# ChrisHekmanOtoy/opencl_render

Hardware: AMD Instinct MI355X
Metric: Mrays/s (primary rays; each also traces its shadow/bounce rays) at ms/frame = ms_per_step (higher is better)
Workload: dtype f32

## Files before the change

### opencl_render_amd/csrc/rt_wavefront.hip

```cpp
#include "rt_devfuncs.h"
#include "rt_launch.h"
#include "rt_ray_clip.h"

namespace {

enum { WS_RAY = 0, WS_SHADOW = 1 };

__device__ __forceinline__ float4 pack4(V3 v, float w) { return make_float4(v.x, v.y, v.z, w); }
__device__ __forceinline__ V3 xyz(float4 v) { return mk(v.x, v.y, v.z); }

__device__ __forceinline__ void store_single_sample(const RtDevScene &S, uint32_t localPixel, V3 c)
{
    const uint32_t slot = localPixel / RT_TILE_PIXELS, inTile = localPixel % RT_TILE_PIXELS;
    uint16_t *planes = S.tileBuf + (size_t)slot * 3 * RT_TILE_PIXELS + inTile;
    uint32_t samples = S.sampleDivisor;
    asm volatile("" : "+s"(samples));
    const float scale = (float)(0xFFFF) / (float)samples;
    planes[0] = (uint16_t)sat_add_u16(0, c.x, scale);
    planes[RT_TILE_PIXELS] = (uint16_t)sat_add_u16(0, c.y, scale);
    planes[2 * RT_TILE_PIXELS] = (uint16_t)sat_add_u16(0, c.z, scale);
}

__device__ __forceinline__ uint32_t wave_append(uint32_t *counter, bool want)
{
    const unsigned long long mask = __ballot(want);
    if (mask == 0) return 0;
    const uint32_t lane = __lane_id();
    const int leader = __ffsll((long long)mask) - 1;
    uint32_t base = 0;
    if ((int)lane == leader) base = atomicAdd(counter, (uint32_t)__popcll(mask));
    base = __shfl(base, leader, 64);
    return base + (uint32_t)__popcll(mask & ((1ull << lane) - 1ull));
}

__device__ __forceinline__ void wave_append2(uint32_t *counterA, bool wantA, uint32_t *counterB, bool wantB, uint32_t &posA, uint32_t &posB)
{
    const unsigned long long maskA = __ballot(wantA), maskB = __ballot(wantB);
    const uint32_t lane = __lane_id();
    uint32_t base = 0;
    const uint32_t n = (lane == 0u) ? (uint32_t)__popcll(maskA) : (uint32_t)__popcll(maskB);
    if (lane < 2u && n != 0u) base = atomicAdd(lane == 0u ? counterA : counterB, n);
    const unsigned long long below = (1ull << lane) - 1ull;
    posA = (uint32_t)__shfl((int)base, 0, 64) + (uint32_t)__popcll(maskA & below);
    posB = (uint32_t)__shfl((int)base, 1, 64) + (uint32_t)__popcll(maskB & below);
}

__device__ __forceinline__ bool tri_rec_test_flat(const float4 r0, const float4 r1, const float4 r2, const float4 r3, V3 o, V3 d, float tmin,
                                                  float tmax, float &t, float &l1, float &l2)
{
    const V3 a = mk(r0.x, r0.y, r0.z), ab = mk(r0.w, r1.x, r1.y), ac = mk(r1.z, r1.w, r2.x), n = mk(r2.y, r2.z, r2.w);
    const V3 ao = sub3(o, a);
    t = -dot3(n, ao) / dot3(n, d);
    const V3 ap = sub3(along(o, t, d), a);
    const float ap_ab = dot3(ap, ab);
    const float ap_ac = dot3(ap, ac);
    l1 = (r3.y * ap_ac - r3.z * ap_ab) * r3.w;
    l2 = (r3.y * ap_ab - r3.x * ap_ac) * r3.w;
    return (tmin < t) & (t < tmax) & (0 <= l1) & (0 <= l2) & (l1 + l2 <= 1.f);
}
// ... 78 lines not shown
}

#if defined(RT_DIAG_STAMPS) || defined(RT_DIAG_LOGIC)
__device__ __forceinline__ unsigned long long diag_stamp()
{
    unsigned long long t;
    asm volatile("s_memtime %0\n\ts_waitcnt lgkmcnt(0)" : "=s"(t)::"memory");
    return t;
}
#endif

}

template <bool PASSES>
__device__ __forceinline__ void wf_primary_body(const RtDevScene &S, const RtWavefront &W, uint32_t *passBuf)
{
    const uint32_t slot = blockIdx.x >> 6, patch = blockIdx.x & 63;
    const uint32_t lane = threadIdx.x & 63, wave = threadIdx.x >> 6;
    const uint32_t lx = (patch & 7) * RT_PATCH + (wave & 1) * 8 + (lane & 7);
    const uint32_t ly = (patch >> 3) * RT_PATCH + (wave >> 1) * 8 + (lane >> 3);
    const uint32_t tile = S.tileIds[slot];
    const uint32_t gx = (tile % S.tilesX) * RT_TILE + lx;
    const uint32_t gy = (tile / S.tilesX) * RT_TILE + ly;
    const uint32_t sb = blockIdx.y;
    const bool valid = gx < S.width && gy < S.height;

    uint32_t hit_tri = RT_NONE;
    float hit_t = 0.f, hit_l1 = 0.f, hit_l2 = 0.f;
    uint64_t rng = 0;
    V3 dir = mk(0.f, 0.f, 0.f);
    const uint32_t localPixel = slot * RT_TILE_PIXELS + ly * RT_TILE + lx;
    const uint32_t outSlot = localPixel * W.samplesInBatch + sb;
    if (valid) {
        const uint32_t pixel = gy * S.width + gx;
        rng = (uint64_t)pixel * (uint64_t)S.seedStride + (uint64_t)(S.sampleFirst + W.sampleBase + sb + 1);
        const V3 lr = ld3(S.lr), tb = ld3(S.tb);
        dir = ld3(S.topLeft);
        float k = (float)gx + rand01(rng);
        dir.x += lr.x * k; dir.y += lr.y * k; dir.z += lr.z * k;
        k = (float)gy + rand01(rng);
        dir.x += tb.x * k; dir.y += tb.y * k; dir.z += tb.z * k;
        hit_tri = camera_scan(S, localPixel, ld3(S.eye), dir, 0.f, RT_INF, RT_NONE, hit_t, hit_l1, hit_l2);
        if (hit_tri == RT_NONE) {
            if (S.directStore == 1u) store_single_sample(S, localPixel, mk(0.f, 0.f, 0.f));
            else W.sampleOut[outSlot] = make_float4(0.f, 0.f, 0.f, 0.f);
        }
    }
    const bool born = valid && hit_tri != RT_NONE;
    const uint32_t shard = (blockIdx.x + blockIdx.y * gridDim.x) % RT_WF_SHARDS;
    const uint32_t a = shard * W.shardCap + wave_append(&W.ctl[RT_WF_CTL_COUNTS + shard], born);
    if (born) {
        W.rng[a] = rng;
        W.meta[a] = make_uint4(outSlot, localPixel, 0u | (1u << 4) | ((uint32_t)WS_RAY << 8), hit_tri);
        W.ring[(size_t)a * (RT_RING * 3) + 1] = pack4(dir, __uint_as_float(RT_NONE));
        W.res[a] = make_uint4(hit_tri, __float_as_uint(hit_t), __float_as_uint(hit_l1), __float_as_uint(hit_l2));
    }
    if (PASSES && valid) {
        uint32_t *pass = passBuf + (size_t)slot * RT_PASS_WORDS * RT_TILE_PIXELS + ly * RT_TILE + lx;
        if (S.sampleCount == 1u) pass[RT_PASS_HITS * RT_TILE_PIXELS] = born ? 1u : 0u;
        else if (born) __hip_atomic_fetch_add(pass + RT_PASS_HITS * RT_TILE_PIXELS, 1u, __ATOMIC_RELAXED, __HIP_MEMORY_SCOPE_AGENT);
        if (W.sampleBase + sb == 0u) {
            const float depth = born ? hit_t * sqrt_rn(dot3(dir, dir)) : RT_INF;
            pass[RT_PASS_DEPTH * RT_TILE_PIXELS] = __float_as_uint(depth);
            pass[RT_PASS_TRIANGLE * RT_TILE_PIXELS] = hit_tri;
        }
    }
}

__global__ __launch_bounds__(256) void wf_primary_kernel(const RtDevScene S, const RtWavefront W) { wf_primary_body<false>(S, W, nullptr); }
__global__ __launch_bounds__(256) void wf_primary_passes_kernel(const RtDevScene S, const RtWavefront W, uint32_t *passBuf)
{
    wf_primary_body<true>(S, W, passBuf);
}

__global__ __launch_bounds__(256) void wf_surface_passes_kernel(const RtDevScene S, const RtWavefront W, float *surfBuf)
{
    __shared__ Shared sh;
    for (int i = threadIdx.x; i < 3 * (RT_GRID_DIV + 1); i += 256) (&sh.planes[0][0])[i] = S.boxMin[i];
    sh.unit255[threadIdx.x] = (float)threadIdx.x / 255.f;
    __syncthreads();
    const uint32_t slot = blockIdx.x >> 6, patch = blockIdx.x & 63;
    const uint32_t lane = threadIdx.x & 63, wave = threadIdx.x >> 6;
    const uint32_t lx = (patch & 7) * RT_PATCH + (wave & 1) * 8 + (lane & 7);
    const uint32_t ly = (patch >> 3) * RT_PATCH + (wave >> 1) * 8 + (lane >> 3);
    const uint32_t tile = S.tileIds[slot];
    const uint32_t gx = (tile % S.tilesX) * RT_TILE + lx;
    const uint32_t gy = (tile / S.tilesX) * RT_TILE + ly;
    if (gx >= S.width || gy >= S.height) return;

    const uint32_t localPixel = slot * RT_TILE_PIXELS + ly * RT_TILE + lx;
    float *sums = surfBuf + (size_t)slot * RT_SURF_WORDS * RT_TILE_PIXELS + ly * RT_TILE + lx;
    float acc[RT_SURF_WORDS];
#pragma unroll
    for (int k = 0; k < RT_SURF_WORDS; ++k) acc[k] = W.sampleBase == 0u ? 0.f : sums[k * RT_TILE_PIXELS];
    const uint32_t pixel = gy * S.width + gx;
    const V3 eye = ld3(S.eye), lr = ld3(S.lr), tb = ld3(S.tb), topLeft = ld3(S.topLeft);
    Counters cn;
    for (uint32_t sb = 0; sb < W.samplesInBatch; ++sb) {
        uint64_t rng = (uint64_t)pixel * (uint64_t)S.seedStride + (uint64_t)(S.sampleFirst + W.sampleBase + sb + 1);
        V3 dir = topLeft;
        float k = (float)gx + rand01(rng);
        dir.x += lr.x * k; dir.y += lr.y * k; dir.z += lr.z * k;
        k = (float)gy + rand01(rng);
        dir.x += tb.x * k; dir.y += tb.y * k; dir.z += tb.z * k;
        float hit_t = 0.f, hit_l1 = 0.f, hit_l2 = 0.f;
        const uint32_t hit_tri = camera_scan(S, localPixel, eye, dir, 0.f, RT_INF, RT_NONE, hit_t, hit_l1, hit_l2);
        V3 n = mk(0.f, 0.f, 0.f), albedo = mk(0.f, 0.f, 0.f);
// ... 187 lines not shown
    const float4 *sp = reinterpret_cast<const float4 *>(S.triShade + 24 * (size_t)tri);
    const float4 s0 = sp[0], s1 = sp[1], s2 = sp[2], s3 = sp[3], s4 = sp[4], s5 = sp[5];
    row.a = reinterpret_cast<const float4 *>(S.triRec)[4 * (size_t)tri];
    row.v[0] = s0.x; row.v[1] = s0.y; row.v[2] = s0.z; row.v[3] = s0.w; row.v[4] = s1.x; row.v[5] = s1.y; row.v[6] = s1.z; row.v[7] = s1.w;
    row.v[8] = s2.x; row.v[9] = s2.y; row.v[10] = s2.z; row.v[11] = s2.w; row.v[12] = s3.x; row.v[13] = s3.y; row.v[14] = s3.z; row.v[15] = s3.w;
    row.v[16] = s4.x; row.v[17] = s4.y; row.v[18] = s4.z; row.v[19] = s4.w; row.v[20] = s5.x; row.v[21] = s5.y; row.v[22] = s5.z; row.v[23] = s5.w;
    row.tri = tri;
}

template <bool FIRST, bool ORDERED, bool LEAN>
__global__ __launch_bounds__(256, LEAN ? (FIRST ? RT_WF_LOGIC_WAVES_LEAN_FIRST : RT_WF_LOGIC_WAVES_LEAN)
                                       : (FIRST ? (ORDERED ? RT_WF_LOGIC_WAVES_FIRST_ORDERED : RT_WF_LOGIC_WAVES_FIRST) : RT_WF_LOGIC_WAVES)) void wf_logic_kernel(const RtDevScene S, const RtWavefront W, const uint32_t round,
                                                                                                             const uint32_t slicesIn, const RtRoundMode next)
{
    constexpr bool SHADE = false;
    const RtShadeList L{ nullptr, nullptr };
#include "rt_wf_logic_body.h"
}

#ifndef RT_WF_ANSWER_WAVES
#define RT_WF_ANSWER_WAVES 8
#endif
__global__ __launch_bounds__(256, RT_WF_ANSWER_WAVES) void wf_answer_kernel(const RtDevScene S, const RtWavefront W, const uint32_t round, const uint32_t slicesIn,
                                                                            const RtShadeList L, const uint32_t shadeFollows)
{
    const uint32_t in = round & 1;
    const uint32_t *ctlIn = W.ctl + (round % 3) * RT_WF_CTL_WORDS;
    const uint32_t lane = threadIdx.x & 63, wave = threadIdx.x >> 6;
    const uint32_t waveId = (blockIdx.x * 256 + threadIdx.x) >> 6, waves = (gridDim.x * 256) >> 6;
    {
        const uint32_t gid = blockIdx.x * 256 + threadIdx.x;
        if (gid < RT_WF_CTL_WORDS) W.ctl[((round + 2) % 3) * RT_WF_CTL_WORDS + gid] = 0u;
        if (gid < RT_WF_SHARDS) L.count[((round + 2) % 3) * RT_WF_SHARDS + gid] = 0u;
    }
    if (blockIdx.x == gridDim.x - 1 && round < RT_WF_ROUND_LOG) log_round_rays(W, ctlIn, round, lane, wave);
    const uint32_t shard = __builtin_amdgcn_readfirstlane(waveId % slicesIn);
    const uint32_t total = __builtin_amdgcn_readfirstlane(ctlIn[RT_WF_CTL_COUNTS + shard]);
    const uint32_t sliceCapIn = W.capacity / slicesIn;
    uint32_t *listCount = L.count + (round % 3) * RT_WF_SHARDS + shard;
    const float4 lc = S.lightCount != 0u ? make_float4(S.lightCol[0], S.lightCol[1], S.lightCol[2], S.lightHalfAtt[0]) : make_float4(0.f, 0.f, 0.f, 0.f);
    for (uint32_t localChunk = __builtin_amdgcn_readfirstlane(waveId / slicesIn); localChunk * 64 < total; localChunk += waves / slicesIn) {
        const uint32_t local = localChunk * 64 + lane;
        const uint32_t q = shard * sliceCapIn + local;
        bool list = false, odd = false;
        uint32_t a = 0;
        unsigned long long listKey = ~0ull;
        if (local < total) {
            const uint2 who = W.pathOf[in][q];
            a = who.x;
            const unsigned long long key = W.hitKey[in][q];
            unsigned long long laKey = ~0ull;
            if (who.y != 0xffffffffu) laKey = W.hitKey[in][who.y];
            const uint4 meta = W.meta[a];
            V3 out = xyz(W.outc[a]);
            int head = (int)(meta.z & 15u);
            const int tail = (int)((meta.z >> 4) & 15u);
            const uint32_t stage = (meta.z >> 8) & 1u, laState = (meta.z >> 10) & 3u;
            const int laIndex = (int)((meta.z >> 12) & 15u);
            if (laState == 2u) laKey = W.laKey[a];
            bool finished = false;
            if (stage == WS_SHADOW) {
                const float4 sp = W.shP[a], sf = W.shFace[a];
                const float lmax = reinterpret_cast<const float *>(W.ent[in] + 4 * (size_t)q)[11];
                const V3 zero = mk(0.f, 0.f, 0.f);
                V3 face = xyz(sf), atten = mk(1.f, 1.f, 1.f);
                if (key != ~0ull) { atten.x *= zero.x; atten.y *= zero.y; atten.z *= zero.z; }
                class_light_accum(face, sp.w, sf.w != 0.f, lmax, lc, atten);
                class_shade_end(out, xyz(sp), face);
                head = (head + 1) % RT_RING;
                if (head == tail) finished = true;
                else if (laState != 0u && laIndex == head) {
                    if (laKey != ~0ull) { list = true; listKey = laKey; W.outc[a] = pack4(out, 0.f); }
                    else if ((head + 1) % RT_RING == tail) finished = true;
                    else odd = true;
                } else odd = true;
            } else if (laState != 0u) odd = true;
            else if (key != ~0ull) { list = true; listKey = key; }
            else if ((head + 1) % RT_RING == tail) finished = true;
            else odd = true;
            if (finished) {
                if (S.directStore == 1u) store_single_sample(S, meta.y, out);
                else W.sampleOut[meta.x] = pack4(out, 0.f);
            }
        }
        if (__ballot(odd) != 0ull && lane == 0u) atomicOr(W.hostStatus + RT_WF_STATUS_ERROR, RT_WF_ERR_SPLIT);
        if (!shadeFollows && __ballot(list) != 0ull && lane == 0u) atomicOr(W.hostStatus + RT_WF_STATUS_ERROR, RT_WF_ERR_GRID);
        const uint32_t at = wave_append(listCount, list);
        if (list) L.list[shard * sliceCapIn + at] = make_uint4(a, (uint32_t)listKey, (uint32_t)(listKey >> 32), 0u);
    }
}

template <bool ORDERED>
__global__ __launch_bounds__(256, RT_WF_LOGIC_WAVES_LEAN) void wf_shade_kernel(const RtDevScene S, const RtWavefront W, const uint32_t round, const uint32_t slicesIn,
                                                                              const RtRoundMode next, const RtShadeList L)
{
    constexpr bool FIRST = false, LEAN = true, SHADE = true;
#include "rt_wf_logic_body.h"
}

__device__ __forceinline__ uint32_t slice_first(const RtWavefront &W, uint32_t slices, uint32_t s)
{
    const uint32_t kind = (s >= slices) ? 1u : 0u, shard = s - kind * slices;
    return kind * W.capacity + shard * (W.capacity / slices);
}
__device__ __forceinline__ uint32_t slice_count(const uint32_t *ctl, uint32_t slices, uint32_t s)
{
    const uint32_t kind = (s >= slices) ? 1u : 0u, shard = s - kind * slices;
    return ctl[RT_WF_CTL_COUNTS + kind * RT_WF_SHARDS + shard];
}

__global__ __launch_bounds__(256) void wf_scatter_kernel(const RtWavefront W, const uint32_t round, const uint32_t slices)
{
    __shared__ uint32_t base[RT_WF_SORT_BINS * RT_WF_SORT_COPIES];
    __shared__ uint32_t longWave[4];
    uint32_t *ctl = W.ctl + (round % 3) * RT_WF_CTL_WORDS;
    const uint32_t lane = threadIdx.x & 63, wave = threadIdx.x >> 6;
// ... 1164 lines not shown
```

### opencl_render_amd/csrc/rt_wf_logic_body.h

```cpp
    __shared__ Shared sh;
    __shared__ float4 ltPosRadius[RT_WF_LIGHTS_LDS], ltDirSpread[RT_WF_LIGHTS_LDS], ltColHalf[RT_WF_LIGHTS_LDS];
    __shared__ int ltType[RT_WF_LIGHTS_LDS];
    __shared__ uint32_t waveHist[ORDERED ? 4 : 1][RT_WF_SORT_BINS], waveBase[ORDERED ? 4 : 1][RT_WF_SORT_BINS];
    __shared__ uint8_t cellLut[ORDERED ? 3 * 256 : 4];
    __shared__ uint8_t itemOwner[ORDERED ? 4 : 1][2 * 64 * (RT_WF_MAXSEG - 1)];
    __shared__ uint32_t itemWord[ORDERED ? 4 : 1][ORDERED ? 2 * 64 * (RT_WF_MAXSEG - 1) : 1];
    __shared__ float lutScale[3];
    static_assert(RT_WF_SORT_BINS == 64, "one class per lane");
    sh.unit255[threadIdx.x] = (float)threadIdx.x / 255.f;
    if (ORDERED) {
        float *pl = &sh.planes[0][0];
        for (int i = threadIdx.x; i < 3 * (RT_GRID_DIV + 1); i += 256) pl[i] = S.boxMin[i];
        waveHist[threadIdx.x >> 6][threadIdx.x & 63] = 0u;
        if (threadIdx.x < 3 * 256 / 4) reinterpret_cast<uint32_t *>(cellLut)[threadIdx.x] = reinterpret_cast<const uint32_t *>(S.cellLut)[threadIdx.x];
        if (threadIdx.x < 3) lutScale[threadIdx.x] = 256.f / (S.boxMin[threadIdx.x * (RT_GRID_DIV + 1) + RT_GRID_DIV] - S.boxMin[threadIdx.x * (RT_GRID_DIV + 1)]);
    }
    if (threadIdx.x < RT_WF_LIGHTS_LDS && threadIdx.x < S.lightCount) {
        const uint32_t k = threadIdx.x;
        ltType[k] = S.lightType[k];
        ltPosRadius[k] = make_float4(S.lightPos[4 * k], S.lightPos[4 * k + 1], S.lightPos[4 * k + 2], S.lightRadius[k]);
        ltDirSpread[k] = make_float4(S.lightDir[4 * k], S.lightDir[4 * k + 1], S.lightDir[4 * k + 2], S.lightSpread[k]);
        ltColHalf[k] = make_float4(S.lightCol[4 * k], S.lightCol[4 * k + 1], S.lightCol[4 * k + 2], S.lightHalfAtt[k]);
    }
    __syncthreads();
// ... 10 lines not shown

    const uint32_t in = round & 1, outq = in ^ 1;
    const uint32_t *ctlIn = W.ctl + (round % 3) * RT_WF_CTL_WORDS;
    uint32_t *ctlOut = W.ctl + ((round + 1) % 3) * RT_WF_CTL_WORDS;
    const uint32_t lane = threadIdx.x & 63, wave = threadIdx.x >> 6;
    const uint32_t waveId = (blockIdx.x * 256 + threadIdx.x) >> 6, waves = (gridDim.x * 256) >> 6;
    Counters cn;
    if (!SHADE) {
        const uint32_t gid = blockIdx.x * 256 + threadIdx.x;
        if (gid < RT_WF_CTL_WORDS) W.ctl[((round + 2) % 3) * RT_WF_CTL_WORDS + gid] = 0u;
    }
    if (SHADE) {
        if (blockIdx.x == gridDim.x - 1 && wave == 0 && round < RT_WF_ROUND_LOG) {
            static_assert(RT_WF_SHARDS == 256, "four list lengths per lane");
            const uint32_t *c = L.count + (round % 3) * RT_WF_SHARDS;
            uint32_t n = c[lane] + c[64 + lane] + c[128 + lane] + c[192 + lane];
#pragma unroll
            for (int off = 32; off >= 1; off >>= 1) n += __shfl_xor(n, off, 64);
            if (lane == 0) reinterpret_cast<uint32_t *>(W.roundLog + round)[3] = n;
        }
    } else
    if (blockIdx.x == gridDim.x - 1 && round < RT_WF_ROUND_LOG) {
        __shared__ uint32_t sumWave[4], maxWave[4];
        static_assert(RT_WF_QSHARDS == 512, "two queue lengths per thread");
        const uint32_t c0 = ctlIn[RT_WF_CTL_COUNTS + threadIdx.x], c1 = ctlIn[RT_WF_CTL_COUNTS + 256 + threadIdx.x];
        uint32_t n = c0 + c1, m = max(c0, c1);
#pragma unroll
        for (int off = 32; off >= 1; off >>= 1) { n += __shfl_xor(n, off, 64); m = max(m, (uint32_t)__shfl_xor((int)m, off, 64)); }
        if (lane == 0) { sumWave[wave] = n; maxWave[wave] = m; }
        __syncthreads();
        if (threadIdx.x == 0) {
            uint32_t *log = reinterpret_cast<uint32_t *>(W.roundLog + round);
            log[0] = sumWave[0] + sumWave[1] + sumWave[2] + sumWave[3];
            log[1] = max(max(maxWave[0], maxWave[1]), max(maxWave[2], maxWave[3]));
        }
    }
    const bool multiLight = S.lightCount > 1u;
    const float *planes = &sh.planes[0][0];

    const uint32_t shard = __builtin_amdgcn_readfirstlane(waveId % slicesIn);
    const uint32_t total = __builtin_amdgcn_readfirstlane(SHADE ? L.count[(round % 3) * RT_WF_SHARDS + shard] : ctlIn[RT_WF_CTL_COUNTS + shard]);
    const uint32_t sliceCapIn = W.capacity / slicesIn, sliceCapOut = W.capacity / next.slices;
    const uint32_t outShard = shard % next.slices;
    for (uint32_t localChunk = __builtin_amdgcn_readfirstlane(waveId / slicesIn); localChunk * 64 < total; localChunk += waves / slicesIn) {
        const uint32_t local = localChunk * 64 + lane;
        const uint32_t q = shard * sliceCapIn + local;
        const bool live = local < total;
#ifdef RT_DIAG_LOGIC
        unsigned long long dg[12];
        dg[0] = diag_stamp();
        for (int i = 1; i < 12; ++i) dg[i] = 0;
#endif
        bool emit = false, emitLa = false;
        V3 ro = mk(0, 0, 0), rd = mk(0, 0, 0), lo3 = mk(0, 0, 0), ld3v = mk(0, 0, 0);
        float rtmin = 0.f, rtmax = 0.f, latmin = 0.f;
        uint32_t rexcl = RT_NONE, laexcl = RT_NONE, a = 0;

        if (LEAN && live) {
            const V3 zero = mk(0.f, 0.f, 0.f);
            uint32_t res_tri = RT_NONE;
            float res_t = 0.f, res_l1 = 0.f, res_l2 = 0.f;
            unsigned long long key = ~0ull, laKeyEarly = ~0ull;
            if (FIRST) {
                a = q;
                const uint4 r = W.res[q];
                res_tri = r.x; res_t = __uint_as_float(r.y); res_l1 = __uint_as_float(r.z); res_l2 = __uint_as_float(r.w);
            } else if (SHADE) {
                const uint4 listed = L.list[q];
                a = listed.x;
                key = (unsigned long long)listed.y | ((unsigned long long)listed.z << 32);
            } else {
                const uint2 who = W.pathOf[in][q];
                a = who.x;
                key = W.hitKey[in][q];
                if (who.y != 0xffffffffu) laKeyEarly = W.hitKey[in][who.y];
            }
            float4 *ringA = W.ring + (size_t)a * (RT_RING * 3);
            uint64_t rng = W.rng[a];
            const uint4 meta = FIRST ? make_uint4(0u, 0u, 0u | (1u << 4) | ((uint32_t)WS_RAY << 8), res_tri) : W.meta[a];
            V3 out = mk(0.f, 0.f, 0.f);
            float4 c0 = make_float4(0.f, 0.f, 0.f, 0.f), c1 = c0, c2 = c0;
            TriRow row;
            row.tri = RT_NONE;
            if (FIRST) {
                c0 = pack4(ld3(S.eye), 0.f); c1 = ringA[1]; c2 = make_float4(1.f, 1.f, 1.f, __uint_as_float((12u << 1) | 1u));
                load_tri_row(S, res_tri, row);
            } else out = xyz(W.outc[a]);
            uint32_t hit_tri = meta.w;
            int head = (int)(meta.z & 15u), tail = (int)((meta.z >> 4) & 15u);
            const uint32_t stage = (meta.z >> 8) & 1u;
            uint32_t laState = (meta.z >> 10) & 3u;
            int laIndex = (int)((meta.z >> 12) & 15u);
            bool laFetched = false;
            unsigned long long laKey = ~0ull;
            if (SHADE) {
                if (stage == WS_SHADOW) head = (head + 1) % RT_RING;
                laState = 0u;
            }
            if (laState == 1u) { laKey = laKeyEarly; laState = 2u; laFetched = true; }
            else if (laState == 2u) laKey = W.laKey[a];

            V3 cur_o = mk(0, 0, 0), cur_d = mk(0, 0, 0), cur_w = mk(0, 0, 0);
            float cur_tmin = 0.f;
            uint32_t cur_excl = RT_NONE;
            int cur_bounces = 0;
            V3 n = mk(0, 0, 0), where = mk(0, 0, 0), P = mk(0, 0, 0), face = mk(0, 0, 0), toL = mk(0, 0, 0);
            float ndl = 0.f, lmin = 0.f, lmax = 0.f;
            bool front = false, finished = false, rngDirty = false, outDirty = false, shade = false;
            uint32_t emitStage = WS_RAY;
            int firstSpawnSlot = -1;
            float4 firstSpawn0 = make_float4(0.f, 0.f, 0.f, 0.f), firstSpawn1 = firstSpawn0;

            auto take_ray = [&](float4 e0, float4 e1, float4 e2) {
                cur_o = xyz(e0); cur_tmin = e0.w; cur_d = xyz(e1); cur_excl = __float_as_uint(e1.w); cur_w = xyz(e2);
                cur_bounces = (int)(__float_as_uint(e2.w) >> 1);
            };
            auto next_ray = [&]() -> bool {
                head = (head + 1) % RT_RING;
                if (head == tail) { finished = true; return false; }
                take_ray(ringA[head * 3 + 0], ringA[head * 3 + 1], ringA[head * 3 + 2]);
                return true;
            };
            auto emit_ray = [&]() { emit = true; emitStage = WS_RAY; ro = cur_o; rd = cur_d; rtmin = cur_tmin; rtmax = RT_INF; rexcl = cur_excl; };
            auto light_accum = [&](V3 atten) {
                const float mag = __builtin_fabsf(ndl);
                const float4 lc = light_col_half(0);
                const float x = lmax / lc.w;
                const float e = mag * half_falloff(x);
                if ((0.f <= ndl) == front) {
                    face.x += (1.f - face.x) * atten.x * e * lc.x;
                    face.y += (1.f - face.y) * atten.y * e * lc.y;
                    face.z += (1.f - face.z) * atten.z * e * lc.z;
                }
            };
            auto shade_end = [&]() {
                out.x += P.x * face.x;
                out.y += P.y * face.y;
                out.z += P.z * face.z;
                outDirty = true;
            };

            bool advance = false;
            if (FIRST) {
                take_ray(c0, c1, c2);
                shade = res_tri != RT_NONE;
                advance = !shade;
            } else if (!SHADE && stage == WS_SHADOW) {
                const float4 sp = W.shP[a], sf = W.shFace[a];
                P = xyz(sp); ndl = sp.w; face = xyz(sf); front = (sf.w != 0.f);
                lmax = reinterpret_cast<const float *>(W.ent[in] + 4 * (size_t)q)[11];
                V3 atten = mk(1.f, 1.f, 1.f);
                if (key != ~0ull) { atten.x *= zero.x; atten.y *= zero.y; atten.z *= zero.z; }
                light_accum(atten);
                shade_end();
                advance = true;
            } else {
                take_ray(ringA[head * 3 + 0], ringA[head * 3 + 1], ringA[head * 3 + 2]);
                res_tri = resolve_hit(S, key, cur_o, cur_d, cur_tmin, RT_INF, cur_excl, res_t, res_l1, res_l2);
                shade = res_tri != RT_NONE;
                advance = !shade;
            }
            if (advance && next_ray()) {
                if (laState == 2u && laIndex == head) {
                    res_tri = resolve_hit(S, laKey, cur_o, cur_d, cur_tmin, RT_INF, cur_excl, res_t, res_l1, res_l2);
                    laState = 0u;
                    shade = res_tri != RT_NONE;
                    if (!shade && next_ray()) emit_ray();
                } else emit_ray();
            }
            if (shade) {
                hit_tri = res_tri;
                const float *shadeRow = FIRST ? row.v : S.triShade + 24 * (size_t)res_tri;
                const int m = __float_as_int(shadeRow[21]);
                const float *uv = shadeRow + 15;
                where = along(cur_o, res_t, cur_d);
                MatRec mat;
                mat.desc[0] = mat.desc[1] = mat.desc[2] = mat.desc[3] = mat.desc[4] = 0u; mat.m = m;
                if (0 <= m) mat = load_mat(S, m);
                n = shading_normal<false, true>(S, sh, where, cur_o, cur_d, hit_tri, res_l1, res_l2, shadeRow, m, cn, &mat, FIRST ? &row.a : nullptr);
                V3 tex = mk(0, 0, 0);
                const V3 transp = zero, refl = zero, lum = zero;
                if (0 <= m && mat.desc[CH_COLOR]) {
                    uint32_t raw;
                    tex = texel_rec<false>(S, sh, mat, CH_COLOR, uv, res_l1, res_l2, raw, cn);
                }
                out.x += (1.f - out.x) * lum.x * cur_w.x;
                out.y += (1.f - out.y) * lum.y * cur_w.y;
                out.z += (1.f - out.z) * lum.z * cur_w.z;
                outDirty = true;
                front = (dot3(n, cur_d) <= 0.f);
                P.x = (1.f - out.x) * cur_w.x * (1.f - transp.x) * tex.x;
                P.y = (1.f - out.y) * cur_w.y * (1.f - transp.y) * tex.y;
                P.z = (1.f - out.z) * cur_w.z * (1.f - transp.z) * tex.z;
                face = mk(0.1f, 0.1f, 0.1f);
                const int type = S.lightCount != 0u ? light_type(0) : 0;
                SphereRaw raw0;
                raw0.p = mk(0, 0, 0); raw0.len = 1.f; raw0.sq = 0.f;
                if (S.lightCount != 0u && type >= 1 && type <= 9) raw0 = sphere_raw(rng);
                rngDirty = true;
                if (cur_bounces > 0) {
                    const int frontI = front ? 1 : 0;
                    const float total_rt = RT_MAX2(RT_MAX2(refl.x + transp.x, refl.y + transp.y), refl.z + transp.z);
                    const float dif = (total_rt < 1.f) ? 1.f - total_rt : 0.f;
                    const V3 w = mk(cur_w.x * tex.x * dif, cur_w.y * tex.y * dif, cur_w.z * tex.z * dif);
                    if (3.f / 256.f <= w.x + w.y + w.z) {
                        V3 nd = sphere_scaled(sphere_raw(rng), 1.f);
                        if (frontI != ((0 <= dot3(nd, n)) ? 1 : 0)) { nd.x = -nd.x; nd.y = -nd.y; nd.z = -nd.z; }
                        const float4 s0 = pack4(where, 0.f), s1 = pack4(nd, __uint_as_float(hit_tri));
                        ringA[tail * 3 + 0] = s0; ringA[tail * 3 + 1] = s1; ringA[tail * 3 + 2] = pack4(w, __uint_as_float(0u));
                        if (FIRST) { firstSpawnSlot = tail; firstSpawn0 = s0; firstSpawn1 = s1; }
                        tail = (tail + 1) % RT_RING;
                    }
                }
                if (S.lightCount != 0u) {
                    toL = mk(0.f, 0.f, 0.f);
                    lmin = 0.f; lmax = 0.f;
                    if (type >= 1 && type <= 9) {
                        if (type >= 3 && type <= 6) {
                            const float4 ld = light_dir_spread(0);
                            toL = sphere_scaled(raw0, ld.w);
                            toL.x -= ld.x; toL.y -= ld.y; toL.z -= ld.z;
                            const float inv = 1.f / sqrt_rn(dot3(toL, toL));
                            toL.x *= inv; toL.y *= inv; toL.z *= inv;
                            lmax = RT_INF;
                        } else {
                            const float4 lp = light_pos_radius(0);
                            const V3 rp = sphere_scaled(raw0, lp.w);
                            toL.x = rp.x + lp.x - where.x;
                            toL.y = rp.y + lp.y - where.y;
                            toL.z = rp.z + lp.z - where.z;
                            lmax = sqrt_rn(dot3(toL, toL));
                            const float inv = 1.f / lmax;
                            toL.x *= inv; toL.y *= inv; toL.z *= inv;
                        }
                    }
                    ndl = dot3(n, toL);
                    const bool dead = W.deadShadow && ((0.f <= ndl) != front);
                    if (lmin < lmax && !dead) { emit = true; emitStage = WS_SHADOW; ro = where; rd = toL; rtmin = lmin; rtmax = lmax; rexcl = hit_tri; }
                    else light_accum(mk(1.f, 1.f, 1.f));
                }
                if (!emit) {
                    shade_end();
                    if (FIRST && firstSpawnSlot >= 0) {
                        head = firstSpawnSlot;
                        emit = true; emitStage = WS_RAY; ro = xyz(firstSpawn0); rtmin = firstSpawn0.w; rd = xyz(firstSpawn1); rtmax = RT_INF;
                        rexcl = __float_as_uint(firstSpawn1.w);
                    } else if (next_ray()) emit_ray();
                }
            }

            if (!finished && laState == 0u && W.lookAhead) {
                const int nx = (head + 1) % RT_RING;
                if (nx != tail) {
                    float4 n0 = firstSpawn0, n1 = firstSpawn1;
                    if (!FIRST || nx != firstSpawnSlot) { n0 = ringA[nx * 3 + 0]; n1 = ringA[nx * 3 + 1]; }
                    emitLa = true; lo3 = xyz(n0); latmin = n0.w; ld3v = xyz(n1); laexcl = __float_as_uint(n1.w);
                    laState = 1u; laIndex = nx;
                }
            }

            if (finished) {
                const uint2 where2 = FIRST ? *reinterpret_cast<const uint2 *>(W.meta + a) : make_uint2(meta.x, meta.y);
                if (S.directStore == 1u) store_single_sample(S, where2.y, out);
                else W.sampleOut[where2.x] = pack4(out, 0.f);
            } else {
                asm volatile("" : "+v"(a));
                if (rngDirty) W.rng[a] = rng;
                if (outDirty) W.outc[a] = pack4(out, 0.f);
                const uint32_t flags = (uint32_t)head | ((uint32_t)tail << 4) | (emitStage << 8) | (laState << 10) | ((uint32_t)laIndex << 12);
                if (FIRST) reinterpret_cast<uint2 *>(W.meta + a)[1] = make_uint2(flags, hit_tri);
                else W.meta[a] = make_uint4(meta.x, meta.y, flags, hit_tri);
                if (laState == 2u && laFetched) W.laKey[a] = laKey;
                if (emitStage == WS_SHADOW) {
                    W.shP[a] = pack4(P, ndl);
                    W.shFace[a] = pack4(face, front ? 1.f : 0.f);
                }
            }
        } else if (live) {
            uint32_t res_tri = RT_NONE;
            float res_t = 0.f, res_l1 = 0.f, res_l2 = 0.f;
            unsigned long long key = ~0ull, laKeyEarly = ~0ull;
            float4 qo = make_float4(0.f, 0.f, 0.f, 0.f), qd = qo;
            if (FIRST) {
                a = q;
                const uint4 r = W.res[q];
                res_tri = r.x; res_t = __uint_as_float(r.y); res_l1 = __uint_as_float(r.z); res_l2 = __uint_as_float(r.w);
            } else {
                const uint2 who = W.pathOf[in][q];
                a = who.x;
                key = W.hitKey[in][q];
                if (who.y != 0xffffffffu) laKeyEarly = W.hitKey[in][who.y];
            }
            float4 *ringA = W.ring + (size_t)a * (RT_RING * 3);
            uint64_t rng = W.rng[a];
            const uint4 meta = FIRST ? make_uint4(0u, 0u, 0u | (1u << 4) | ((uint32_t)WS_RAY << 8), res_tri) : W.meta[a];
            V3 out = mk(0.f, 0.f, 0.f);
            float4 c0 = qo, c1 = qo, c2 = qo;
            unsigned long long laKey = ~0ull;
            TriRow row;
            row.tri = RT_NONE;
            if (FIRST) {
                c0 = pack4(ld3(S.eye), 0.f); c1 = ringA[1]; c2 = make_float4(1.f, 1.f, 1.f, __uint_as_float((12u << 1) | 1u));
                load_tri_row(S, res_tri, row);
            } else out = xyz(W.outc[a]);
            uint32_t hit_tri = meta.w;
            int head = (int)(meta.z & 15u), tail = (int)((meta.z >> 4) & 15u);
            const uint32_t stage = (meta.z >> 8) & 1u;
            bool attStored = ((meta.z >> 9) & 1u) != 0u;
            uint32_t laState = (meta.z >> 10) & 3u;
            int laIndex = (int)((meta.z >> 12) & 15u);
            uint32_t j = meta.z >> 16;
            DG(1);
            bool laFetched = false;
            if (laState == 1u) { laKey = laKeyEarly; laState = 2u; laFetched = true; }
            else if (laState == 2u) laKey = W.laKey[a];

            V3 cur_o = mk(0, 0, 0), cur_d = mk(0, 0, 0), cur_w = mk(0, 0, 0);
            float cur_tmin = 0.f;
            uint32_t cur_excl = RT_NONE;
            int cur_bounces = 0, cur_fromCamera = 0;
            V3 n = mk(0, 0, 0), where = mk(0, 0, 0), P = mk(0, 0, 0), face = mk(0, 0, 0), atten = mk(1.f, 1.f, 1.f), toL = mk(0, 0, 0);
// ... 199 lines not shown
                        pc = PC_RAY_RESULT;
                    } else if (laState == 2u && laIndex == head) {
                        res_tri = resolve_hit(S, laKey, cur_o, cur_d, cur_tmin, RT_INF, cur_excl, res_t, res_l1, res_l2);
                        laState = 0u;
                        pc = PC_RAY_RESULT;
                    } else {
                        emit = true; emitStage = WS_RAY; ro = cur_o; rd = cur_d; rtmin = cur_tmin; rtmax = RT_INF; rexcl = cur_excl;
                        pc = PC_EXIT;
                    }
                }
            }

            DG(6);
            if (!finished && laState == 0u && W.lookAhead) {
                const int nx = (head + 1) % RT_RING;
                if (nx != tail) {
                    float4 n0 = firstSpawn0, n1 = firstSpawn1;
                    uint32_t nflags = firstSpawnFlags;
                    if (!FIRST || nx != firstSpawnSlot) { n0 = ringA[nx * 3 + 0]; n1 = ringA[nx * 3 + 1]; nflags = __float_as_uint(ringA[nx * 3 + 2].w); }
                    if ((nflags & 1u) == 0u) {
                        emitLa = true; lo3 = xyz(n0); latmin = n0.w; ld3v = xyz(n1); laexcl = __float_as_uint(n1.w);
                        laState = 1u; laIndex = nx;
                    }
                }
            }

            if (laexcl != 12345u) DG(7);
            if (finished) {
                const uint2 where2 = FIRST ? *reinterpret_cast<const uint2 *>(W.meta + a) : make_uint2(meta.x, meta.y);
                if (S.directStore == 1u) store_single_sample(S, where2.y, out);
                else W.sampleOut[where2.x] = pack4(out, 0.f);
            } else {
                asm volatile("" : "+v"(a));
                if (rngDirty) W.rng[a] = rng;
                if (outDirty) W.outc[a] = pack4(out, 0.f);
                const uint32_t flags = (uint32_t)head | ((uint32_t)tail << 4) | (emitStage << 8) | ((attStored ? 1u : 0u) << 9) | (laState << 10) |
                                       ((uint32_t)laIndex << 12) | (j << 16);
                if (FIRST) reinterpret_cast<uint2 *>(W.meta + a)[1] = make_uint2(flags, hit_tri);
                else W.meta[a] = make_uint4(meta.x, meta.y, flags, hit_tri);
                if (laState == 2u && laFetched) W.laKey[a] = laKey;
                if (emitStage == WS_SHADOW) {
                    W.shP[a] = pack4(P, ndl);
                    W.shFace[a] = pack4(face, front ? 1.f : 0.f);
                    if (attStored) W.shAtt[a] = pack4(atten, 0.f);
                    if (multiLight) {
                        W.rngL[a] = rngL;
                        if (shadedNow) W.shN[a] = pack4(n, 0.f);
                    }
                }
            }
        }
        uint32_t slot, slotLa;
        wave_append2(&ctlOut[RT_WF_CTL_COUNTS + outShard], emit, &ctlOut[RT_WF_CTL_COUNTS + RT_WF_SHARDS + outShard], emitLa, slot, slotLa);
        slot += outShard * sliceCapOut;
        slotLa += W.capacity + outShard * sliceCapOut;
        asm volatile("" : "+v"(a), "+v"(slot), "+v"(slotLa));
        if (slot != 0xfffffff0u) DG(8);
        const uint32_t copy = waveId % RT_WF_SORT_COPIES;
        if (!ORDERED) {
#pragma unroll 1
            for (int which = 0; which < 2; ++which) {
                const bool has = which ? emitLa : emit;
                if (!has) continue;
                const V3 o = which ? lo3 : ro, d = which ? ld3v : rd;
                const float tmin = which ? latmin : rtmin, tmax = which ? RT_INF : rtmax;
                const uint32_t excluded = which ? laexcl : rexcl, mine = which ? slotLa : slot;
                uint4 *e = W.ent[outq] + 4 * (size_t)mine;
                if (!which) W.pathOf[outq][mine] = make_uint2(a, emitLa ? slotLa : 0xffffffffu);
                W.hitKey[outq][mine] = ~0ull;
                reinterpret_cast<uint32_t *>(e)[3] = excluded;
                reinterpret_cast<uint32_t *>(e)[7] = __float_as_uint(tmin);
                e[2] = make_uint4(__float_as_uint(o.x), __float_as_uint(o.y), __float_as_uint(o.z), __float_as_uint(tmax));
                e[3] = make_uint4(__float_as_uint(d.x), __float_as_uint(d.y), __float_as_uint(d.z), 0u);
            }
        } else {
            auto visit_class = [](uint32_t v) -> uint32_t {
                if ((int)v < 1) v = 1;
                if (v > 767u) v = 767u;
                return (v < 128u) ? 63u - (v >> 2) : 31u - (v - 128u) / 20u;
            };
            EntryPlan planM, planL;
            planM.visits = planL.visits = 1; planM.endCell = planL.endCell = 0xffffffffu; planM.te = planL.te = RT_INF;
            planM.start.cell = planL.start.cell = 0; planM.start.dx = planM.start.dy = planM.start.dz = 0.f; planL.start.dx = planL.start.dy = planL.start.dz = 0.f;
            uint32_t nsegM = 0, nsegL = 0;
            const uint8_t *lut = next.segLen >= 4096u ? cellLut : nullptr;
#pragma unroll 1
            for (int which = 0; which < 2; ++which) {
                const bool has = which ? emitLa : emit;
                if (__ballot(has) == 0ull) continue;
                const V3 o = which ? lo3 : ro, d = which ? ld3v : rd;
                const float tmin = which ? latmin : rtmin, tmax = which ? RT_INF : rtmax;
                const bool sameStart = which && emit && lo3.x == ro.x && lo3.y == ro.y && lo3.z == ro.z && latmin == 0.f && rtmin == 0.f &&
                                       planes[0] <= o.x && o.x <= planes[RT_GRID_DIV] && planes[RT_GRID_DIV + 1] <= o.y && o.y <= planes[2 * RT_GRID_DIV + 1] &&
                                       planes[2 * (RT_GRID_DIV + 1)] <= o.z && o.z <= planes[3 * RT_GRID_DIV + 2];
                if (has) {
                    const EntryPlan plan = plan_ray(planes, o, d, tmin, tmax, sameStart, planM.start.cell, lut, lutScale, S.boxMin + RT_CLIP_AT);
                    const uint32_t n = segments_of(plan, d, tmax, next.segLen);
                    if (which) { planL = plan; nsegL = n; } else { planM = plan; nsegM = n; }
                }
            }
            const uint32_t extraM = nsegM > 1u ? nsegM - 1u : 0u, extraL = nsegL > 1u ? nsegL - 1u : 0u;
            uint32_t itemsM = 0, itemsL = 0, beforeM = 0, beforeL = 0;
            const bool cutting = __ballot((extraM | extraL) != 0u) != 0ull;
            if (cutting) {
                uint32_t inclM = extraM, inclL = extraL;
#pragma unroll
// ... 157 lines not shown
```

Measured before the change: 2785.

## Compact per-path ring storage for opaque-diffuse class and park lmax in outc

For the opaque-diffuse path class, the 12-slot per-path ray ring is replaced by a compact layout: slot 0 holds the primary direction and a single bounce slot holds spawned bounce rays, cutting the per-path memory footprint and scattered traffic. The shadow-stage light max distance is now stored in the w component of the outc record instead of being re-read from the entry queue, and outc is written unconditionally. Paths that would need a ring slot other than the bounce slot set a split-error status flag in the lean kernel. This relies on the path class guaranteeing at most one pending bounce ray, and it adds an extra outc store on every non-finished path.

```diff
diff --git a/opencl_render_amd/csrc/rt_path_state.h b/opencl_render_amd/csrc/rt_path_state.h
--- /dev/null
+++ b/opencl_render_amd/csrc/rt_path_state.h
@@ -0,0 +1,24 @@
+#ifndef RT_PATH_STATE_H
+#define RT_PATH_STATE_H
+
+#include <stddef.h>
+#include <stdint.h>
+
+#if defined(__HIPCC__) || defined(__CUDACC__)
+#define RT_PATH_HD __host__ __device__ __forceinline__
+#else
+#define RT_PATH_HD inline
+#endif
+
+#define RT_PATH_RING_SLOTS 12
+#define RT_PATH_RING_QUADS (RT_PATH_RING_SLOTS * 3)
+#define RT_PATH_CLASS_BOUNCE_SLOT 1u
+
+RT_PATH_HD size_t rt_path_ring_quad(uint32_t a, uint32_t slot, uint32_t quad) { return (size_t)a * RT_PATH_RING_QUADS + slot * 3u + quad; }
+
+RT_PATH_HD size_t rt_path_class_quad(uint32_t capacity, uint32_t a, uint32_t slot, uint32_t quad)
+{
+    return slot == 0u ? (size_t)a : (size_t)capacity + 4u * (size_t)a + quad;
+}
+
+#endif
diff --git a/opencl_render_amd/csrc/rt_wavefront.hip b/opencl_render_amd/csrc/rt_wavefront.hip
--- a/opencl_render_amd/csrc/rt_wavefront.hip
+++ b/opencl_render_amd/csrc/rt_wavefront.hip
@@ -1,10 +1,12 @@
 #include "rt_devfuncs.h"
 #include "rt_launch.h"
+#include "rt_path_state.h"
 #include "rt_ray_clip.h"
 
 namespace {
 
 enum { WS_RAY = 0, WS_SHADOW = 1 };
+static_assert(RT_PATH_RING_SLOTS == RT_RING, "rt_path_state.h addresses the ring allocation");
 
 __device__ __forceinline__ float4 pack4(V3 v, float w) { return make_float4(v.x, v.y, v.z, w); }
 __device__ __forceinline__ V3 xyz(float4 v) { return mk(v.x, v.y, v.z); }
@@ -189,7 +191,8 @@
     if (born) {
         W.rng[a] = rng;
         W.meta[a] = make_uint4(outSlot, localPixel, 0u | (1u << 4) | ((uint32_t)WS_RAY << 8), hit_tri);
-        W.ring[(size_t)a * (RT_RING * 3) + 1] = pack4(dir, __uint_as_float(RT_NONE));
+        const size_t dirAt = S.pathClass == RT_PATH_CLASS_OPAQUE_DIFFUSE ? rt_path_class_quad(W.capacity, a, 0u, 1u) : rt_path_ring_quad(a, 0u, 1u);
+        W.ring[dirAt] = pack4(dir, __uint_as_float(RT_NONE));
         W.res[a] = make_uint4(hit_tri, __float_as_uint(hit_t), __float_as_uint(hit_l1), __float_as_uint(hit_l2));
     }
     if (PASSES && valid) {
@@ -483,7 +486,8 @@
             unsigned long long laKey = ~0ull;
             if (who.y != 0xffffffffu) laKey = W.hitKey[in][who.y];
             const uint4 meta = W.meta[a];
-            V3 out = xyz(W.outc[a]);
+            const float4 oc = W.outc[a];
+            V3 out = xyz(oc);
             int head = (int)(meta.z & 15u);
             const int tail = (int)((meta.z >> 4) & 15u);
             const uint32_t stage = (meta.z >> 8) & 1u, laState = (meta.z >> 10) & 3u;
@@ -492,7 +496,7 @@
             bool finished = false;
             if (stage == WS_SHADOW) {
                 const float4 sp = W.shP[a], sf = W.shFace[a];
-                const float lmax = reinterpret_cast<const float *>(W.ent[in] + 4 * (size_t)q)[11];
+                const float lmax = oc.w;
                 const V3 zero = mk(0.f, 0.f, 0.f);
                 V3 face = xyz(sf), atten = mk(1.f, 1.f, 1.f);
                 if (key != ~0ull) { atten.x *= zero.x; atten.y *= zero.y; atten.z *= zero.z; }
diff --git a/opencl_render_amd/csrc/rt_wf_logic_body.h b/opencl_render_amd/csrc/rt_wf_logic_body.h
--- a/opencl_render_amd/csrc/rt_wf_logic_body.h
+++ b/opencl_render_amd/csrc/rt_wf_logic_body.h
@@ -86,6 +86,7 @@
         for (int i = 1; i < 12; ++i) dg[i] = 0;
 #endif
         bool emit = false, emitLa = false;
+        bool odd = false;
         V3 ro = mk(0, 0, 0), rd = mk(0, 0, 0), lo3 = mk(0, 0, 0), ld3v = mk(0, 0, 0);
         float rtmin = 0.f, rtmax = 0.f, latmin = 0.f;
         uint32_t rexcl = RT_NONE, laexcl = RT_NONE, a = 0;
@@ -109,17 +110,25 @@
                 key = W.hitKey[in][q];
                 if (who.y != 0xffffffffu) laKeyEarly = W.hitKey[in][who.y];
             }
-            float4 *ringA = W.ring + (size_t)a * (RT_RING * 3);
+            auto bounce_of = [&]() -> float4 * {
+                uint32_t path = a;
+                asm volatile("" : "+v"(path));
+                return W.ring + rt_path_class_quad(W.capacity, path, RT_PATH_CLASS_BOUNCE_SLOT, 0u);
+            };
             uint64_t rng = W.rng[a];
             const uint4 meta = FIRST ? make_uint4(0u, 0u, 0u | (1u << 4) | ((uint32_t)WS_RAY << 8), res_tri) : W.meta[a];
             V3 out = mk(0.f, 0.f, 0.f);
+            float parkedLmax = 0.f;
             float4 c0 = make_float4(0.f, 0.f, 0.f, 0.f), c1 = c0, c2 = c0;
             TriRow row;
             row.tri = RT_NONE;
             if (FIRST) {
-                c0 = pack4(ld3(S.eye), 0.f); c1 = ringA[1]; c2 = make_float4(1.f, 1.f, 1.f, __uint_as_float((12u << 1) | 1u));
+                c0 = pack4(ld3(S.eye), 0.f); c1 = W.ring[rt_path_class_quad(W.capacity, a, 0u, 1u)]; c2 = make_float4(1.f, 1.f, 1.f, __uint_as_float((12u << 1) | 1u));
                 load_tri_row(S, res_tri, row);
-            } else out = xyz(W.outc[a]);
+            } else {
+                const float4 oc = W.outc[a];
+                out = xyz(oc); parkedLmax = oc.w;
+            }
             uint32_t hit_tri = meta.w;
             int head = (int)(meta.z & 15u), tail = (int)((meta.z >> 4) & 15u);
             const uint32_t stage = (meta.z >> 8) & 1u;
@@ -140,7 +149,7 @@
             int cur_bounces = 0;
             V3 n = mk(0, 0, 0), where = mk(0, 0, 0), P = mk(0, 0, 0), face = mk(0, 0, 0), toL = mk(0, 0, 0);
             float ndl = 0.f, lmin = 0.f, lmax = 0.f;
-            bool front = false, finished = false, rngDirty = false, outDirty = false, shade = false;
+            bool front = false, finished = false, rngDirty = false, shade = false;
             uint32_t emitStage = WS_RAY;
             int firstSpawnSlot = -1;
             float4 firstSpawn0 = make_float4(0.f, 0.f, 0.f, 0.f), firstSpawn1 = firstSpawn0;
@@ -152,7 +161,9 @@
             auto next_ray = [&]() -> bool {
                 head = (head + 1) % RT_RING;
                 if (head == tail) { finished = true; return false; }
-                take_ray(ringA[head * 3 + 0], ringA[head * 3 + 1], ringA[head * 3 + 2]);
+                odd |= head != (int)RT_PATH_CLASS_BOUNCE_SLOT;
+                const float4 *bounce = bounce_of();
+                take_ray(bounce[0], bounce[1], bounce[2]);
                 return true;
             };
             auto emit_ray = [&]() { emit = true; emitStage = WS_RAY; ro = cur_o; rd = cur_d; rtmin = cur_tmin; rtmax = RT_INF; rexcl = cur_excl; };
@@ -171,7 +182,6 @@
                 out.x += P.x * face.x;
                 out.y += P.y * face.y;
                 out.z += P.z * face.z;
-                outDirty = true;
             };
 
             bool advance = false;
@@ -182,14 +192,16 @@
             } else if (!SHADE && stage == WS_SHADOW) {
                 const float4 sp = W.shP[a], sf = W.shFace[a];
                 P = xyz(sp); ndl = sp.w; face = xyz(sf); front = (sf.w != 0.f);
-                lmax = reinterpret_cast<const float *>(W.ent[in] + 4 * (size_t)q)[11];
+                lmax = parkedLmax;
                 V3 atten = mk(1.f, 1.f, 1.f);
                 if (key != ~0ull) { atten.x *= zero.x; atten.y *= zero.y; atten.z *= zero.z; }
                 light_accum(atten);
                 shade_end();
                 advance = true;
             } else {
-                take_ray(ringA[head * 3 + 0], ringA[head * 3 + 1], ringA[head * 3 + 2]);
+                odd |= head != (int)RT_PATH_CLASS_BOUNCE_SLOT;
+                const float4 *bounce = bounce_of();
+                take_ray(bounce[0], bounce[1], bounce[2]);
                 res_tri = resolve_hit(S, key, cur_o, cur_d, cur_tmin, RT_INF, cur_excl, res_t, res_l1, res_l2);
                 shade = res_tri != RT_NONE;
                 advance = !shade;
@@ -221,7 +233,6 @@
                 out.x += (1.f - out.x) * lum.x * cur_w.x;
                 out.y += (1.f - out.y) * lum.y * cur_w.y;
                 out.z += (1.f - out.z) * lum.z * cur_w.z;
-                outDirty = true;
                 front = (dot3(n, cur_d) <= 0.f);
                 P.x = (1.f - out.x) * cur_w.x * (1.f - transp.x) * tex.x;
                 P.y = (1.f - out.y) * cur_w.y * (1.f - transp.y) * tex.y;
@@ -241,7 +252,9 @@
                         V3 nd = sphere_scaled(sphere_raw(rng), 1.f);
                         if (frontI != ((0 <= dot3(nd, n)) ? 1 : 0)) { nd.x = -nd.x; nd.y = -nd.y; nd.z = -nd.z; }
                         const float4 s0 = pack4(where, 0.f), s1 = pack4(nd, __uint_as_float(hit_tri));
-                        ringA[tail * 3 + 0] = s0; ringA[tail * 3 + 1] = s1; ringA[tail * 3 + 2] = pack4(w, __uint_as_float(0u));
+                        odd |= tail != (int)RT_PATH_CLASS_BOUNCE_SLOT;
+                        float4 *bounce = bounce_of();
+                        bounce[0] = s0; bounce[1] = s1; bounce[2] = pack4(w, __uint_as_float(0u));
                         if (FIRST) { firstSpawnSlot = tail; firstSpawn0 = s0; firstSpawn1 = s1; }
                         tail = (tail + 1) % RT_RING;
                     }
@@ -287,7 +300,11 @@
                 const int nx = (head + 1) % RT_RING;
                 if (nx != tail) {
                     float4 n0 = firstSpawn0, n1 = firstSpawn1;
-                    if (!FIRST || nx != firstSpawnSlot) { n0 = ringA[nx * 3 + 0]; n1 = ringA[nx * 3 + 1]; }
+                    if (!FIRST || nx != firstSpawnSlot) {
+                        odd |= nx != (int)RT_PATH_CLASS_BOUNCE_SLOT;
+                        const float4 *bounce = bounce_of();
+                        n0 = bounce[0]; n1 = bounce[1];
+                    }
                     emitLa = true; lo3 = xyz(n0); latmin = n0.w; ld3v = xyz(n1); laexcl = __float_as_uint(n1.w);
                     laState = 1u; laIndex = nx;
                 }
@@ -300,7 +317,7 @@
             } else {
                 asm volatile("" : "+v"(a));
                 if (rngDirty) W.rng[a] = rng;
-                if (outDirty) W.outc[a] = pack4(out, 0.f);
+                W.outc[a] = pack4(out, rtmax);
                 const uint32_t flags = (uint32_t)head | ((uint32_t)tail << 4) | (emitStage << 8) | (laState << 10) | ((uint32_t)laIndex << 12);
                 if (FIRST) reinterpret_cast<uint2 *>(W.meta + a)[1] = make_uint2(flags, hit_tri);
                 else W.meta[a] = make_uint4(meta.x, meta.y, flags, hit_tri);
@@ -606,6 +623,7 @@
         }
         uint32_t slot, slotLa;
         wave_append2(&ctlOut[RT_WF_CTL_COUNTS + outShard], emit, &ctlOut[RT_WF_CTL_COUNTS + RT_WF_SHARDS + outShard], emitLa, slot, slotLa);
+        if (LEAN && __ballot(odd) != 0ull && lane == 0u) atomicOr(W.hostStatus + RT_WF_STATUS_ERROR, RT_WF_ERR_SPLIT);
         slot += outShard * sliceCapOut;
         slotLa += W.capacity + outShard * sliceCapOut;
         asm volatile("" : "+v"(a), "+v"(slot), "+v"(slotLa));
```

Result: faster. 2896, median of 6 (+4.0%).
